# cure-lab/MotionCraft

Measured on AMD Instinct MI355X. Metric: sampled SMPL-X frames/sec (196-frame seq, 1000-step DDPM), higher is better.
Workload: dtype f32

## Files before the change

include/motioncraft_amd.h:

```cpp
#ifndef MOTIONCRAFT_AMD_H
#define MOTIONCRAFT_AMD_H
#include <stdint.h>

#ifdef __cplusplus
extern "C" {
#endif

#define MC_OK 0
#define MC_ERR_ARG 1
#define MC_ERR_HIP 2
#define MC_ERR_STATE 3
#define MC_ERR_NOCONV 4

typedef struct mc_model mc_model;
typedef struct mc_ctx mc_ctx;

typedef struct mc_model_config {
    int32_t input_feats;
    int32_t max_seq_len;
    int32_t latent_dim;
    int32_t num_parts;
    int32_t num_layers;
    int32_t ffn_dim;
    int32_t time_embed_dim;
// ... 116 lines not shown
int mc_op_temporal_attention(const float* mf_dev, const float* tf_dev, const float* mask_dev, float* yt_dev, int32_t b0, int32_t nb,
                             int32_t B, int32_t T, int32_t Nt, int32_t H, int32_t L, int32_t form, int32_t skip_text,
                             const int32_t* twin_flag_dev, void* stream);
enum { MC_ENC_ATTN_LAYER = 0,
       MC_ENC_ATTN_SMALL = 1,
       MC_ENC_ATTN_STREAM = 2 };
int mc_op_enc_ln(const float* x_dev, const float* gamma_dev, const float* beta_dev, float* y_dev, int64_t rows, int32_t L, float eps,
                 int32_t relu, void* stream);
int mc_op_enc_embed_tokens(const int32_t* ids_dev, const float* emb_dev, const float* pos_dev, float* x_dev, int64_t rows, int32_t S,
                           int32_t d, int32_t vocab, void* stream);
int mc_op_enc_attention(const float* qkv_dev, const uint8_t* valid_dev, float* out_dev, int32_t B, int32_t S, int32_t d, int32_t heads,
                        int32_t causal, int32_t form, void* stream);
enum { MC_GM_PLAIN = 0, MC_GM_ENC = 4 };
typedef struct mc_gemm_strided {
    const float* a_dev; int64_t lda, a_gstride;
    const float* w_dev; int64_t ldw, w_gstride;
    const float* bias_dev; int64_t b_gstride;
    float* c_dev; int64_t ldc, c_gstride;
    const float* res_dev; int64_t ldr, r_gstride;
    const float* add_dev; int64_t ld_add, dup_rows;
    int32_t add_mod, act, act_after_res, M, N, K;
} mc_gemm_strided;
int mc_op_gemm_strided(int32_t mode, int32_t groups, const mc_gemm_strided* args, void* stream);
int mc_op_bigru_steps(const float* gi_dev, const float* whh_dev, const float* bhh_dev, float* h_dev, const int32_t* lens_dev,
                      int32_t len_div, int32_t B, int32_t S, int32_t H, int32_t s0, int32_t steps, void* stream);
int mc_op_conv1d_k4s2(const float* x_dev, int64_t ldx, const float* w_tapmajor_dev, const float* bias_dev, float* y_padded_dev, int32_t B,
                      int32_t T, int32_t C, int32_t Cp, int32_t O, float slope, void* stream);
int mc_op_sampler_update(const float* x_t_dev, const float* out_text_dev, const float* out_none_dev,
                         const float* noise_dev, float* x_prev_dev, float* x0_dev, int64_t n,
                         const mc_step_coefs* coefs, void* stream);

#define MC_POST_MAXTAP 129
int mc_postprocess_smplx(const float* pred_dev, const int32_t* lengths_dev, const double* mean_dev,
                         const double* std_dev, const double* taps_dev, const int32_t radius[4], int32_t stats_f32,
                         int32_t B, int32_t T, int32_t C, double* poses_dev, double* expr_dev, double* trans_dev,
                         void* stream);
int mc_postprocess_smplx_stitched(const float* pred_dev, const int32_t* rows_dev, int32_t n_frames,
                                  const double* mean_dev, const double* std_dev, const double* taps_dev,
                                  const int32_t radius[4], int32_t stats_f32, int32_t C, double* poses_dev,
                                  double* expr_dev, double* trans_dev, void* stream);

int mc_postprocess_t2m_joints(const float* pred_dev, const int32_t* lengths_dev, const double* mean_dev,
                              const double* std_dev, const double* taps_dev, int32_t radius, int32_t stats_f32,
                              int32_t B, int32_t T, int32_t C, int32_t joints_num, float* joints_out_dev, void* stream);
int mc_postprocess_t2m_joints_stitched(const float* pred_dev, const int32_t* rows_dev, int32_t n_frames,
                                       const double* mean_dev, const double* std_dev, const double* taps_dev,
// ... 204 lines not shown
```

motioncraft_amd/csrc/mc_ctx.h:

```cpp
#pragma once
#include <map>
#include <mutex>
#include <string>
#include <vector>

#include "../../include/motioncraft_amd.h"
#include "mc_common.h"
#include "mc_gemm.h"
#include "mc_kernels.h"
#include "mc_chain.h"
#include "mc_half.h"
#include "mc_options.h"
#include "mc_params.h"

struct mc_model {
    mc_model_config cfg;
    ParamStore params{""};
    std::map<std::string, HalfW> half;
    std::mutex half_mu;
    size_t half_bytes = 0;
    bool finalized = false;
    int Cp = 0;
};

struct MoeW {
    const float *emb, *gate_w, *gate_b, *sim_n, *sim_nT, *scale, *fc1_w, *fc1_b, *fc2_wt, *fc2_b, *proj_w, *proj_b;
    int din, dout;
};

struct LayerW {
    const float *norm_g, *norm_b, *tnorm_g, *tnorm_b, *wsm;
    MoeW mm, tm;
    const float *dyn_g, *dyn_b, *qkv_w, *qkv_b;
    const float *ca_film_w, *ca_film_b, *ca_ln_g, *ca_ln_b, *ca_out_w, *ca_out_b;
    const float *ffn_w1, *ffn_b1, *ffn_w2, *ffn_b2;
    const float *ffn_film_w, *ffn_film_b, *ffn_ln_g, *ffn_ln_b, *ffn_out_w, *ffn_out_b;
    const float *before_w = nullptr, *before_b = nullptr, *after_w = nullptr, *after_b = nullptr;
    HalfW h_ca_out, h_ffn_out, h_fc1, h_fc2, h_w1, h_w2, h_after, h_proj, h_qkv;
};

struct ProfRec { hipEvent_t e0 = nullptr, e1 = nullptr; long rows = 0; };

struct mc_ctx {
    mc_model* m = nullptr;
    McOptions opt{};
// ... 80 lines not shown
```

motioncraft_amd/csrc/mc_gemm.h:

```cpp
#pragma once
#include <hip/hip_runtime.h>
#include "mc_options.h"
#include "../../include/motioncraft_amd.h"

enum { GM_PLAIN = MC_GM_PLAIN, GM_EXP1 = 1, GM_EXP2 = 2, GM_COMB = 3, GM_ENC = MC_GM_ENC };

enum : int {
    kTuneStaging = 1 << 0,
    kTuneDma = 1 << 4,
    kTuneWp = 1 << 5,
    kTuneNoXcd = 1 << 6,
    kTuneSmallXcd = 1 << 8,
    kTuneEncWp = 1 << 9,
    kTuneTail2 = 1 << 10,
    kTuneBits = kTuneStaging | kTuneDma | kTuneWp | kTuneNoXcd | kTuneSmallXcd | kTuneEncWp | kTuneTail2,
    kTuneDefault = kTuneBits & ~kTuneNoXcd,
};
static_assert(kTuneDefault == 1841, "the default tune bits are public ABI");

struct GemmArgs {
    const float* A = nullptr;
    long lda = 0;
    int a_col = 0;
    long a_gstride = 0;
    const float* W = nullptr;
    long ldw = 0;
    long w_gstride = 0;
    const float* bias = nullptr;
    long b_gstride = 0;
    float* C = nullptr;
    long ldc = 0;
    int c_col = 0;
    long c_gstride = 0;
    const float* R = nullptr;
    long ldr = 0;
    long r_gstride = -1;
    int act = 0;
    int act_after_res = 0;
    const float* add = nullptr;
    int add_mod = 1;
    long ld_add = 0;
    long dup_rows = 0;
    int M = 0, N = 0, K = 0;
    const int* tile_group = nullptr;
    const int* tile_row0 = nullptr;
    const int* tile_nrows = nullptr;
    const int* num_tiles = nullptr;
    const int* src_row = nullptr;
    const int* dst_row = nullptr;
    const float* comb_w = nullptr;
    int small_tile_n = 0;
    int wp_grid = 0;
    int tune = -1;
};

inline void mc_gemm_opts(const McOptions& o, GemmArgs& g) {
    g.tune = (int)o.gemm_tune;
    g.small_tile_n = o.small_tile_n ? (int)o.small_tile_n : -1;
    g.wp_grid = o.gemm_wp_grid > 0 ? (int)o.gemm_wp_grid : -1;
}

inline double mc_cu_load(long workgroups) {
    const long n = (workgroups + 255) / 256;
    return (1.45 * (double)(n / 2) + (double)(n % 2));
}

int mc_device_cus();
int mc_launch_gemm(int mode, const GemmArgs& g, int groups, int max_tiles, hipStream_t stream);
int mc_launch_gemm_small(const GemmArgs& g, hipStream_t stream, int groups = 1);

struct TailArgs {
    const float* H = nullptr;
    const float* Af = nullptr;
    long half = 0, lda = 0;
    const float* W = nullptr;
    long ldw = 0, w_gstride = 0;
    const float* bias = nullptr;
    long b_gstride = 0;
    float* C = nullptr;
    float* C2 = nullptr;
    long ldc = 0;
    int M = 0, N = 0, K = 0;
    float wc = 1.f, wu = 0.f;
    const float* coef_table = nullptr;
    const int* step_ptr = nullptr;
    long coef_stride = 0;
    int tune = -1;
};
int mc_launch_gemm_tail(const TailArgs& g, hipStream_t stream);
bool mc_gemm_tail_two_outputs(const TailArgs& g);
// ... 1 lines not shown
```

motioncraft_amd/csrc/mc_gemm.hip:

```cpp
#include "mc_common.h"
#include "mc_gemm.h"

namespace {

constexpr int BM = 128, BN = 128, BK = 32, LD = BK + 4;

struct Stage {
    long aoff[4], woff[4];
    bool aok[4], wok[4];
    float cw0[4], cw1[4];
};

template <int MODE, bool GUARD>
__device__ __forceinline__ void load_tile(const GemmArgs& g, const float* __restrict__ Ab, const float* __restrict__ Wb,
                                          const Stage& st, int k, f32x4 (&ra)[4], f32x4 (&rb)[4]) {
    const bool kin = !GUARD || k < g.K;
#pragma unroll
    for (int i = 0; i < 4; ++i) {
        f32x4 v = {0.f, 0.f, 0.f, 0.f};
        if ((!GUARD || st.aok[i]) && kin) {
            if constexpr (MODE == GM_COMB) {
                f32x4 y0 = {0.f, 0.f, 0.f, 0.f}, y1 = {0.f, 0.f, 0.f, 0.f};
                if (st.cw0[i] != 0.f) y0 = *reinterpret_cast<const f32x4*>(Ab + st.aoff[i] + k);
                if (st.cw1[i] != 0.f) y1 = *reinterpret_cast<const f32x4*>(Ab + st.aoff[i] + g.lda + k);
// ... 312 lines not shown
        const float* At = As + buf * BM * BK + (wm * 64 + frow) * BK;
        const float* Bt = Bs + buf * BN * BK + (wn * 64 + frow) * BK;
        Frag f0 = ld_frag(At, Bt, 0);
        Frag f1 = ld_frag(At, Bt, 1);
        __builtin_amdgcn_sched_barrier(0);
        mma(f0);
        f0 = ld_frag(At, Bt, 2);
        __builtin_amdgcn_sched_barrier(0);
        mma(f1);
        f1 = ld_frag(At, Bt, 3);
        __builtin_amdgcn_sched_barrier(0);
        mma(f0);
        mma(f1);
        __syncthreads();
    }
    if (g.act == ACT_GELU) epilogue_vec<GM_PLAIN, false, ACT_GELU>(g, 0, row0, BM, tn, wm, wn, lane, acc);
    else if (g.act == ACT_SILU) epilogue_vec<GM_PLAIN, false, ACT_SILU>(g, 0, row0, BM, tn, wm, wn, lane, acc);
    else if (g.act == ACT_NONE) epilogue_vec<GM_PLAIN, false, ACT_NONE>(g, 0, row0, BM, tn, wm, wn, lane, acc);
    else epilogue_vec<GM_PLAIN, false, ACT_LRELU>(g, 0, row0, BM, tn, wm, wn, lane, acc);
}

constexpr int WBK = 16, WSTAGE = 128 * WBK;

__global__ __launch_bounds__(256, 2) void gemm_wp_k(GemmArgs g) {
    __shared__ __attribute__((aligned(16))) float smem[4 * 2 * WSTAGE];
    const int tid = threadIdx.x, lane = tid & 63, wave = tid >> 6;
    const int wm = wave >> 1, wn = wave & 1;
    const int ntn = g.N / BN, ntiles = (g.M / BM) * ntn;
    const int wave_u = __builtin_amdgcn_readfirstlane(wave);
    float* wbase = smem + wave_u * 2 * WSTAGE;
    const unsigned lds0 = (unsigned)(size_t)wbase;
    const int dr = lane >> 2, dc = ((lane & 3) ^ ((dr >> 2) & 3)) * 4;
    const int frow = lane & 31, hf = lane >> 5, sw = (frow >> 2) & 3;
    const float* Ab = g.A + g.a_col;
    const float* Wb = g.W;
    const float* __restrict__ Rb = g.R ? g.R + g.c_col : nullptr;
    float* __restrict__ Cb = g.C + g.c_col;
    const int nk = g.K / WBK;
    struct Frag { f32x4 a0, a1, b0, b1; };
    auto ld_frag = [&](int st, int j) {
        const float* S = wbase + st * WSTAGE + frow * WBK + ((2 * j + hf) ^ sw) * 4;
        Frag f;
        f.a0 = *reinterpret_cast<const f32x4*>(S);
        f.a1 = *reinterpret_cast<const f32x4*>(S + 32 * WBK);
        f.b0 = *reinterpret_cast<const f32x4*>(S + 64 * WBK);
        f.b1 = *reinterpret_cast<const f32x4*>(S + 96 * WBK);
        return f;
    };
    for (int t = blockIdx.x; t < ntiles; t += gridDim.x) {
        const int bid = (g.tune & kTuneNoXcd) ? t : xcd_remap(t, ntiles);
        const int tm = bid / ntn, tn = bid % ntn;
        const int row0 = tm * BM;
        unsigned voa[4], vow[4];
#pragma unroll
        for (int q = 0; q < 4; ++q) {
            voa[q] = (unsigned)(((long)(row0 + wm * 64 + 16 * q + dr) * g.lda + dc) * 4);
            vow[q] = (unsigned)(((long)(tn * BN + wn * 64 + 16 * q + dr) * g.ldw + dc) * 4);
        }
        auto issue_q = [&](int kt, int st, int q) {
            const unsigned l = lds0 + st * WSTAGE * 4;
            dma16(voa[q], Ab + kt * WBK, l + q * 1024);
            dma16(vow[q], Wb + kt * WBK, l + 4096 + q * 1024);
        };
        f32x16 acc[2][2];
#pragma unroll
        for (int mi = 0; mi < 2; ++mi)
#pragma unroll
            for (int ni = 0; ni < 2; ++ni)
#pragma unroll
                for (int r = 0; r < 16; ++r) acc[mi][ni][r] = 0.f;
        auto mma2 = [&](const Frag& f, int i0) {
#pragma unroll
            for (int i = i0; i < i0 + 2; ++i) {
                acc[0][0] = __builtin_amdgcn_mfma_f32_32x32x2f32(f.b0[i], f.a0[i], acc[0][0], 0, 0, 0);
                acc[0][1] = __builtin_amdgcn_mfma_f32_32x32x2f32(f.b1[i], f.a0[i], acc[0][1], 0, 0, 0);
                acc[1][0] = __builtin_amdgcn_mfma_f32_32x32x2f32(f.b0[i], f.a1[i], acc[1][0], 0, 0, 0);
                acc[1][1] = __builtin_amdgcn_mfma_f32_32x32x2f32(f.b1[i], f.a1[i], acc[1][1], 0, 0, 0);
            }
        };
#pragma unroll
        for (int q = 0; q < 4; ++q) issue_q(0, 0, q);
        asm volatile("s_waitcnt vmcnt(0)" ::: "memory");
        Frag f0 = ld_frag(0, 0);
        auto ktile = [&](int kt) {
            const int st = kt & 1;
            const bool more = kt + 1 < nk;
            Frag f1 = ld_frag(st, 1);
            __builtin_amdgcn_sched_barrier(0);
            mma2(f0, 0);
            if (more) { issue_q(kt + 1, st ^ 1, 0); issue_q(kt + 1, st ^ 1, 1); }
            __builtin_amdgcn_sched_barrier(0);
            mma2(f0, 2);
            if (more) { issue_q(kt + 1, st ^ 1, 2); issue_q(kt + 1, st ^ 1, 3); }
            __builtin_amdgcn_sched_barrier(0);
            mma2(f1, 0);
            if (more) {
                asm volatile("s_waitcnt vmcnt(0)" ::: "memory");
                f0 = ld_frag(st ^ 1, 0);
            }
            __builtin_amdgcn_sched_barrier(0);
            mma2(f1, 2);
        };
        const int npre = nk > 2 ? nk - 2 : 0;
        for (int kt = 0; kt < npre; ++kt) ktile(kt);
        f32x4 rv[2][2][4], bv[2][4];
#pragma unroll
        for (int ni = 0; ni < 2; ++ni)
#pragma unroll
            for (int q = 0; q < 4; ++q) {
                const int n = tn * BN + wn * 64 + ni * 32 + 8 * q + 4 * hf;
                bv[ni][q] = g.bias ? *reinterpret_cast<const f32x4*>(g.bias + n) : f32x4{0.f, 0.f, 0.f, 0.f};
#pragma unroll
                for (int mi = 0; mi < 2; ++mi) {
                    const long m = row0 + wm * 64 + mi * 32 + frow;
                    rv[mi][ni][q] = Rb ? *reinterpret_cast<const f32x4*>(Rb + m * g.ldr + n) : f32x4{0.f, 0.f, 0.f, 0.f};
                    if (g.add) rv[mi][ni][q] = *reinterpret_cast<const f32x4*>(g.add + (m % g.add_mod) * g.ld_add + n);
                }
            }
        for (int kt = npre; kt < nk; ++kt) ktile(kt);
#pragma unroll
        for (int mi = 0; mi < 2; ++mi) {
            float* crow = Cb + (long)(row0 + wm * 64 + mi * 32 + frow) * g.ldc;
#pragma unroll
            for (int ni = 0; ni < 2; ++ni)
#pragma unroll
                for (int q = 0; q < 4; ++q) {
                    const int n = tn * BN + wn * 64 + ni * 32 + 8 * q + 4 * hf;
                    f32x4 v = {acc[mi][ni][4 * q], acc[mi][ni][4 * q + 1], acc[mi][ni][4 * q + 2], acc[mi][ni][4 * q + 3]};
                    v += bv[ni][q];
                    if (g.act != ACT_NONE) {
#pragma unroll
                        for (int jj = 0; jj < 4; ++jj) v[jj] = apply_act(v[jj], g.act);
                    }
                    v += rv[mi][ni][q];
                    *reinterpret_cast<f32x4*>(crow + n) = v;
                    if (g.dup_rows) *reinterpret_cast<f32x4*>(crow + g.dup_rows * g.ldc + n) = v;
                }
        }
    }
}

constexpr int SM = 64, SN = 64, SRING = 4;
template <bool VEC>
__global__ __launch_bounds__(256) void gemm_small_k(GemmArgs g) {
    __shared__ __attribute__((aligned(16))) float smem[SRING * 2 * SM * BK];
    const int tid = threadIdx.x, lane = tid & 63, wave = tid >> 6;
    const int wm = wave >> 1, wn = wave & 1;
    const int ntn = (g.N + SN - 1) / SN;
    const int bid = (g.tune & kTuneSmallXcd) ? xcd_remap((int)blockIdx.x, (int)gridDim.x) : (int)blockIdx.x;
    const int tm = bid / ntn, tn = bid % ntn, grp = blockIdx.y;
    const int row0 = tm * SM;
    const int wave_u = __builtin_amdgcn_readfirstlane(wave);
    const int dr = lane >> 3, dc = ((lane & 7) ^ dr) * 4;
    const float* Ab = g.A + (long)grp * g.a_gstride + g.a_col;
    const float* Wb = g.W + (long)grp * g.w_gstride;
    unsigned voa[2], vow[2];
#pragma unroll
    for (int q = 0; q < 2; ++q) {
        const int ar = min(row0 + 16 * wave + 8 * q + dr, g.M - 1), wr = min(tn * SN + 16 * wave + 8 * q + dr, g.N - 1);
        voa[q] = (unsigned)(((long)ar * g.lda + dc) * 4);
        vow[q] = (unsigned)(((long)wr * g.ldw + dc) * 4);
    }
// ... 510 lines not shown
    int nb = SN;
    double best = cost(SN, 30.0);
    const bool any_width = g.M > 6400;
    if ((g.N % 48 == 0 || any_width) && cost(48, 23.0) < 0.97 * best) { nb = 48; best = cost(48, 23.0); }
    if ((g.N % 96 == 0 || any_width) && cost(96, 41.0) < 0.97 * best) { nb = 96; best = cost(96, 41.0); }
    if (gg.small_tile_n == 64 || gg.small_tile_n == 48 || gg.small_tile_n == 96) nb = gg.small_tile_n;
    dim3 grid(cdiv(g.M, SM) * cdiv(g.N, nb), ng);
    const bool vec16 = vec && g.N % nb == 0;
    MC_LEDGER(nb == 48 ? "gemm_small16_k<3" : nb == 96 ? "gemm_small16_k<6" : "gemm_small_k", grid, 2.0 * g.M * g.N * g.K * ng);
    if (nb == 48) {
        if (vec16) hipLaunchKernelGGL((gemm_small16_k<3, true>), grid, dim3(256), 0, stream, gg);
        else hipLaunchKernelGGL((gemm_small16_k<3, false>), grid, dim3(256), 0, stream, gg);
    } else if (nb == 96) {
        if (vec16) hipLaunchKernelGGL((gemm_small16_k<6, true>), grid, dim3(256), 0, stream, gg);
        else hipLaunchKernelGGL((gemm_small16_k<6, false>), grid, dim3(256), 0, stream, gg);
    } else {
        if (vec) hipLaunchKernelGGL(gemm_small_k<true>, grid, dim3(256), 0, stream, gg);
        else hipLaunchKernelGGL(gemm_small_k<false>, grid, dim3(256), 0, stream, gg);
    }
    MC_LAUNCH_CHECK();
    return MC_OK;
}

int mc_launch_gemm(int mode, const GemmArgs& g0, int groups, int max_tiles, hipStream_t stream) {
    GemmArgs g = g0;
    if (int r = resolve_opts(g)) return r;
    const int ntn = cdiv(g.N, BN);
    int ntm = (mode == GM_EXP1 || mode == GM_EXP2) ? max_tiles : cdiv(g.M, BM);
    if (ntm <= 0 || ntn <= 0) return MC_OK;
    if (mode != GM_ENC) MC_REQUIRE(g.K % 4 == 0 && g.lda % 4 == 0 && g.ldw % 4 == 0, "gemm: K/lda/ldw must be multiples of 4");
    if (mode == GM_ENC && (g.add || g.dup_rows))
        MC_REQUIRE(g.N % 4 == 0 && g.ldc % 4 == 0 && g.c_col % 4 == 0 && g.c_gstride % 4 == 0 && (!g.add || g.ld_add % 4 == 0) &&
                       (!g.R || (g.ldr % 4 == 0 && (g.r_gstride < 0 || g.r_gstride % 4 == 0))),
                   "gemm: an add table or duplicate rows need 16-byte aligned output rows (N=%d ldc=%ld)", g.N, g.ldc);
    dim3 grid(ntm * ntn, groups > 0 ? groups : 1, 1);
    const bool vec_out = (g.ldc % 4 == 0) && (g.c_col % 4 == 0) && (!g.R || g.ldr % 4 == 0);
    const bool wp_ok = (g.tune & kTuneWp) && g.K % WBK == 0 && (long)g.M * g.lda * 4 < (1L << 32) && (long)g.N * g.ldw * 4 < (1L << 32);
    const bool enc_fast = mode == GM_ENC && (g.tune & kTuneEncWp) && wp_ok && !g.R && g.add && g.ld_add % 4 == 0 && g.act == ACT_NONE;
    if ((g.tune & kTuneDma) && (mode == GM_PLAIN || enc_fast) && groups <= 1 && g.M % BM == 0 && g.N % BN == 0 && (g.K % BK == 0 || enc_fast) &&
        g.lda % 4 == 0 && g.ldw % 4 == 0 && g.a_col % 4 == 0 && vec_out && g.act != ACT_QUICKGELU && !g.act_after_res &&
        (enc_fast || (!g.add && !g.dup_rows))) {
        if (wp_ok) {
            const int persistent = g.wp_grid > 0 ? g.wp_grid : (int)grid.x;
            MC_LEDGER("gemm_wp_k", dim3(grid.x < persistent ? grid.x : persistent), 2.0 * g.M * g.N * g.K);
            hipLaunchKernelGGL(gemm_wp_k, dim3(grid.x < persistent ? grid.x : persistent), dim3(256), 0, stream, g);
        } else {
            MC_LEDGER("gemm_dma_k", grid, 2.0 * g.M * g.N * g.K);
            hipLaunchKernelGGL(gemm_dma_k, grid, dim3(256), 0, stream, g);
        }
        MC_LAUNCH_CHECK();
        return MC_OK;
    }
    if (mc_ledger_on) {
        char name[24];
        snprintf(name, sizeof(name), "gemm_k<%d>", mode);
        const double rows = (mode == GM_EXP1 || mode == GM_EXP2) ? (double)ntm * BM : (double)g.M;
        MC_LEDGER(name, grid, 2.0 * rows * g.N * g.K * (groups > 0 ? groups : 1));
    }
    switch (mode) {
        case GM_PLAIN: hipLaunchKernelGGL(gemm_k<GM_PLAIN>, grid, dim3(256), 0, stream, g); break;
        case GM_EXP1: hipLaunchKernelGGL(gemm_k<GM_EXP1>, grid, dim3(256), 0, stream, g); break;
        case GM_EXP2: hipLaunchKernelGGL(gemm_k<GM_EXP2>, grid, dim3(256), 0, stream, g); break;
        case GM_COMB: hipLaunchKernelGGL(gemm_k<GM_COMB>, grid, dim3(256), 0, stream, g); break;
        case GM_ENC: hipLaunchKernelGGL(gemm_k<GM_ENC>, grid, dim3(256), 0, stream, g); break;
        default: mc_set_error("bad gemm mode %d", mode); return MC_ERR_ARG;
    }
    MC_LAUNCH_CHECK();
// ... 75 lines not shown
```

motioncraft_amd/csrc/mc_model.hip:

```cpp
#include "mc_ctx.h"

namespace {

template <class T>
int ws_alloc(mc_ctx* c, T** p, size_t n) {
    void* d = nullptr;
    size_t bytes = (n * sizeof(T) + 255) & ~(size_t)255;
    if (bytes == 0) bytes = 256;
    MC_HIP(hipMalloc(&d, bytes));
    c->allocs.push_back(d);
    c->bytes += (int64_t)bytes;
    *p = (T*)d;
    return MC_OK;
}

int bind_moe(const mc_model* m, const std::string& pre, int din, int dout, int seq_rows, MoeW* w) {
    const int64_t E = m->cfg.num_experts;
    w->din = din;
    w->dout = dout;
    return m->params.bind({{&w->emb, pre + "emb", (int64_t)seq_rows * din},       {&w->gate_w, pre + "gate_w", 256 * din},
                           {&w->gate_b, pre + "gate_b", 256},                      {&w->sim_n, pre + "sim_n", 256 * E},
                           {&w->sim_nT, pre + "sim_nT", 32 * 256},                 {&w->scale, pre + "scale", 1},
                           {&w->fc1_w, pre + "fc1_w", E * 4 * din * din},          {&w->fc1_b, pre + "fc1_b", E * 4 * din},
                           {&w->fc2_wt, pre + "fc2_wt", E * din * 4 * din},        {&w->fc2_b, pre + "fc2_b", E * din},
// ... 216 lines not shown
    MC_REQUIRE(cfg && out, "null argument");
    MC_REQUIRE(cfg->latent_dim == 32 || cfg->latent_dim == 64 || cfg->latent_dim == 128,
               "latent_dim=%d unsupported (32, 64, 128)", cfg->latent_dim);
    MC_REQUIRE(cfg->topk == 2, "topk=%d unsupported (reference configs use 2)", cfg->topk);
    MC_REQUIRE(cfg->num_experts >= 2 && cfg->num_experts <= 16, "num_experts=%d unsupported", cfg->num_experts);
    MC_REQUIRE(cfg->latent_dim % cfg->dyn_heads == 0, "latent_dim %% dyn_heads != 0");
    MC_REQUIRE(cfg->num_ctrl_layers >= 0 && cfg->num_ctrl_layers < cfg->num_layers, "copy_blocks_num=%d must be in [0, num_layers)", cfg->num_ctrl_layers);
    MC_REQUIRE(cfg->num_ctrl_layers == 0 || cfg->ctrl_cond_feats >= 1, "ctrl_cond_feats must be >= 1");
    MC_REQUIRE(cfg->ffn_dim % 4 == 0 && cfg->time_embed_dim % 4 == 0 && cfg->text_latent_dim % 4 == 0, "dims must be multiples of 4");
    {
        const int q = cfg->text_latent_dim / 4;
        MC_REQUIRE(q >= 1 && q <= 64 && (q & (q - 1)) == 0, "text_latent_dim=%d unsupported", cfg->text_latent_dim);
    }
    mc_model* m = new mc_model();
    m->cfg = *cfg;
    m->Cp = (cfg->input_feats + 31) / 32 * 32;
    *out = m;
    return MC_OK;
}

void mc_model_destroy(mc_model* m) {
    if (!m) return;
    for (auto& kv : m->half) (void)hipFree(const_cast<mc_half*>(kv.second.hi));
    delete m;
}

int mc_model_set_param(mc_model* m, const char* name, const float* host, int64_t numel) {
    MC_REQUIRE(m && name && host && numel > 0, "bad argument");
    MC_REQUIRE(!m->finalized || !m->params.has(name), "mc_model_set_param(%s): the model is finalized; weights are immutable from then on", name);
    return m->params.set(name, host, numel);
}

int mc_model_finalize(mc_model* m) {
    MC_REQUIRE(m, "null model");
    mc_ctx probe;
    probe.m = m;
    int r = bind_weights(&probe);
    if (r != MC_OK) return r;
    m->finalized = true;
    return MC_OK;
}

int mc_ctx_create(mc_model* m, int32_t batch, int32_t frames, int32_t max_steps, mc_ctx** out) {
    MC_REQUIRE(m && out, "null argument");
    MC_REQUIRE(m->finalized, "model not finalized");
    MC_REQUIRE(batch >= 1 && frames >= 1 && frames <= m->cfg.max_seq_len, "bad batch/frames (%d, %d)", batch, frames);
    MC_REQUIRE(max_steps >= 1, "max_steps < 1");
    const mc_model_config& g = m->cfg;
    mc_ctx* c = new mc_ctx();
    if (int r = seed_options(c->opt)) { mc_ctx_destroy(c); return r; }
    c->m = m;
    c->B = batch;
    c->T = frames;
// ... 484 lines not shown
int mc_op_gemm(const float* a, const float* w, const float* bias, const float* res, float* cdev, int32_t M, int32_t N,
               int32_t K, int32_t ldw, int32_t act, void* stream) {
    MC_REQUIRE(a && w && cdev && M > 0 && N > 0 && K > 0 && K % 4 == 0 && ldw % 4 == 0 && ldw >= K, "bad gemm args");
    return dense(nullptr, a, K, w, ldw, bias, res, N, cdev, N, M, N, K, act, (hipStream_t)stream);
}

int mc_op_gemm_strided(int32_t mode, int32_t groups, const mc_gemm_strided* a, void* stream) {
    MC_REQUIRE(a && (mode == GM_PLAIN || mode == GM_ENC) && groups >= 1, "gemm_strided: mode %d (0 plain, 4 encoder), groups %d", mode, groups);
    MC_REQUIRE(a->a_dev && a->w_dev && a->c_dev && a->M > 0 && a->N > 0 && a->K > 0 && a->lda > 0 && a->ldc >= a->N && a->ldw >= a->K &&
                   a->ldw % 4 == 0 && a->add_mod >= 1 && a->dup_rows >= 0 && (!a->res_dev || a->ldr >= a->N) && (!a->add_dev || a->ld_add >= a->N),
               "bad gemm_strided args");
    GemmArgs g;
    g.A = a->a_dev; g.lda = a->lda; g.a_gstride = a->a_gstride;
    g.W = a->w_dev; g.ldw = a->ldw; g.w_gstride = a->w_gstride;
    g.bias = a->bias_dev; g.b_gstride = a->b_gstride;
    g.C = a->c_dev; g.ldc = a->ldc; g.c_gstride = a->c_gstride;
    g.R = a->res_dev; g.ldr = a->ldr; g.r_gstride = a->r_gstride;
    g.act = a->act; g.act_after_res = a->act_after_res;
    g.add = a->add_dev; g.add_mod = a->add_mod; g.ld_add = a->ld_add; g.dup_rows = a->dup_rows;
    g.M = a->M; g.N = a->N; g.K = a->K;
    return mc_launch_gemm(mode, g, groups, 0, (hipStream_t)stream);
}

static int gemm_f16_op(GemmHArgs g, const float* w, const float* bias, const float* res, float* cdev, int M, int N, int K, bool split, hipStream_t s) {
    mc_half* planes = nullptr;
    MC_HIP(hipMalloc((void**)&planes, sizeof(mc_half) * 2 * (size_t)N * K));
    int r = mc_launch_split_f16(w, planes, planes + (size_t)N * K, (long)N * K, s);
    if (r == MC_OK) {
        g.Wh = planes; g.Wl = planes + (size_t)N * K; g.bias = bias; g.R = res; g.ldr = N; g.C = cdev; g.ldc = N;
        g.M = M; g.N = N; g.K = K;
        r = mc_launch_gemm_h(g, split, s);
    }
    (void)hipStreamSynchronize(s);
    (void)hipFree(planes);
    return r;
}

int mc_op_gemm_f16(const float* a, const float* w, const float* bias, const float* res, float* cdev, int32_t M, int32_t N,
                   int32_t K, int32_t split, void* stream) {
    MC_REQUIRE(a && w && cdev && M > 0 && N > 0 && K > 0, "bad gemm args");
    GemmHArgs g;
    g.A = a; g.lda = K;
    return gemm_f16_op(g, w, bias, res, cdev, M, N, K, split != 0, (hipStream_t)stream);
}

int mc_op_gemm_f16_planes(const void* a_hi, const void* a_lo, const float* w, const float* bias, const float* res, float* cdev, int32_t M,
// ... 80 lines not shown
```

motioncraft_amd/csrc/mc_step.hip:

```cpp
#include "mc_ctx.h"

bool use_half(const mc_ctx* c) { return c->prec != MC_PREC_F32 && c->rows > c->opt.half_min_rows; }
static const HalfW* half_planes(const mc_ctx* c, const HalfW* hw) { return hw && hw->hi && use_half(c) ? hw : nullptr; }
static bool split3(const mc_ctx* c) { return c->prec == MC_PREC_F16X3; }

static bool twin_aliased(const mc_ctx* c, bool twin) { return twin && chain_on(c, kChainTwinAlias) && !c->no_alias; }
static TwinAlias twin_alias(const mc_ctx* c, bool twin, bool tokens) {
    return twin_aliased(c, twin) ? TwinAlias{mc_route_split_flag_ptr(c->rb), (tokens ? c->N : c->rows) / 2} : TwinAlias();
}

template <class Args>
static void set_tile_map(const mc_ctx* c, int group, Args& a) {
    const long to = (long)group * c->rb.max_tiles;
    a.tile_group = c->rb.tile_group + to; a.tile_row0 = c->rb.tile_row0 + to; a.tile_nrows = c->rb.tile_nrows + to;
    a.num_tiles = mc_route_num_tiles_ptr(c->rb, group);
}

static int dbg_hold(const mc_ctx* c, hipStream_t pos, hipStream_t neg) {
    const long us = c->opt.dbg_delay_us;
    return us == 0 ? MC_OK : mc_launch_spin((us > 0 ? us : -us) * 100, us > 0 ? pos : neg);
}

int dense(const mc_ctx* c, const float* A, long lda, const float* W, long ldw, const float* bias, const float* R, long ldr,
          float* C, long ldc, long M, int N, int K, int act, hipStream_t s) {
// ... 474 lines not shown
int denoise_impl(mc_ctx* c, const float* x_t, int32_t step, float* out2_dev, int32_t stop_after, void* stream, const SeedArgs* seed) {
    MC_REQUIRE(c && x_t, "null argument");
    MC_REQUIRE(c->have_cond, "mc_ctx_set_condition not called");
    MC_REQUIRE(step >= 0 && step < c->S, "step_index %d outside the %d-step schedule", step, c->S);
    if (c->graph_mode) step = 0;
    hipStream_t s = (hipStream_t)stream;
    const mc_model_config& g = c->m->cfg;
    const int L = g.latent_dim, H = g.num_parts, D = L * H, C = g.input_feats;
    const long BT = (long)c->B * c->T;
    int r;
    if ((r = pick_side_stream(c, s))) return r;
    {
        const bool padded = c->xpad_ready && !seed;
        c->xpad_ready = false;
        if (seed) { if ((r = mc_launch_pad_rows_seeded(const_cast<float*>(x_t), c->xpad, BT, C, c->m->Cp, *seed, s))) return r; }
        else if (!padded && (r = mc_launch_pad_rows(x_t, c->xpad, BT, C, c->m->Cp, s))) return r;
        GemmArgs e;
        mc_gemm_opts(c->opt, e);
        e.A = c->xpad; e.lda = c->m->Cp;
        e.W = c->enc_w; e.ldw = c->m->Cp; e.bias = c->enc_b;
        e.add = c->seq_emb; e.add_mod = c->T; e.ld_add = D;
        e.C = c->h; e.ldc = D; e.dup_rows = BT;
        e.M = (int)BT; e.N = D; e.K = c->m->Cp;
        if (BT <= c->opt.small_gemm_rows && D % 64 == 0 && c->m->Cp % 32 == 0) { if ((r = mc_launch_gemm_small(e, s))) return r; }
        else if ((r = mc_launch_gemm(GM_ENC, e, 1, 0, s))) return r;
    }
    const int nl = stop_after >= 0 ? (stop_after < g.num_layers ? stop_after : g.num_layers) : g.num_layers;
    c->no_alias = stop_after >= 0 && stop_after < g.num_layers;
    const int NC = c->have_ctrl ? g.num_ctrl_layers : 0;
    const bool fused = chain_on(c, kChainGate) && chain_on(c, kChainRowchain) && mc_mlp_supported(L, 32);
    const int split = (c->side && chain_on(c, kChainTwoStreams) && c->N > c->opt.big_tokens && fused) ? ((NC > 0 && !chain_on(c, kChainCtrlGroups)) ? 1 : 2) : 0;
    auto by_group = [&](auto&& fn) -> int {
        if (split != 2) return fn(0L, c->rows, s);
        if (int e = fn(0L, BT, s)) return e;
        return fn(BT, BT, c->side);
    };
    for (int i = 0; i < nl; ++i) {
        if (i >= 1 && i <= NC) {
            const int j = i - 1, slot = g.num_layers + j;
            if (j == 0) {
                if ((r = by_group([&](long r0, long n, hipStream_t sk) {
                         return mc_launch_add_rows(c->hc + r0 * D, c->h + r0 * D, c->cb + r0 * D, nullptr, n, D, sk); })))
                    return r;
            }
            if ((r = run_layer(c, slot, c->hc, step, false, split, s))) return r;
            const LayerW& cw = c->lw[slot];
            if ((r = by_group([&](long r0, long n, hipStream_t sk) {
// ... 80 lines not shown
```

Before: 661.1.

## Skip all-zero weight K-tiles in encoder GEMM and split remainder tiles in half

```diff
diff --git a/include/motioncraft_amd.h b/include/motioncraft_amd.h
--- a/include/motioncraft_amd.h
+++ b/include/motioncraft_amd.h
@@ -162,6 +162,7 @@
     int32_t add_mod, act, act_after_res, M, N, K;
 } mc_gemm_strided;
 int mc_op_gemm_strided(int32_t mode, int32_t groups, const mc_gemm_strided* args, void* stream);
+int mc_op_gemm_wp(int32_t mode, const mc_gemm_strided* args, int32_t wp_grid, int64_t tune, int32_t klist, void* stream);
 int mc_op_bigru_steps(const float* gi_dev, const float* whh_dev, const float* bhh_dev, float* h_dev, const int32_t* lens_dev,
                       int32_t len_div, int32_t B, int32_t S, int32_t H, int32_t s0, int32_t steps, void* stream);
 int mc_op_conv1d_k4s2(const float* x_dev, int64_t ldx, const float* w_tapmajor_dev, const float* bias_dev, float* y_padded_dev, int32_t B,
diff --git a/motioncraft_amd/csrc/mc_ctx.h b/motioncraft_amd/csrc/mc_ctx.h
--- a/motioncraft_amd/csrc/mc_ctx.h
+++ b/motioncraft_amd/csrc/mc_ctx.h
@@ -21,6 +21,7 @@
     size_t half_bytes = 0;
     bool finalized = false;
     int Cp = 0;
+    int* enc_klist = nullptr;
 };
 
 struct MoeW {
diff --git a/motioncraft_amd/csrc/mc_gemm.h b/motioncraft_amd/csrc/mc_gemm.h
--- a/motioncraft_amd/csrc/mc_gemm.h
+++ b/motioncraft_amd/csrc/mc_gemm.h
@@ -1,5 +1,6 @@
 #pragma once
 #include <hip/hip_runtime.h>
+#include <vector>
 #include "mc_options.h"
 #include "../../include/motioncraft_amd.h"
 
@@ -13,10 +14,12 @@
     kTuneSmallXcd = 1 << 8,
     kTuneEncWp = 1 << 9,
     kTuneTail2 = 1 << 10,
-    kTuneBits = kTuneStaging | kTuneDma | kTuneWp | kTuneNoXcd | kTuneSmallXcd | kTuneEncWp | kTuneTail2,
+    kTuneEncSkip = 1 << 11,
+    kTuneHalfTiles = 1 << 12,
+    kTuneBits = kTuneStaging | kTuneDma | kTuneWp | kTuneNoXcd | kTuneSmallXcd | kTuneEncWp | kTuneTail2 | kTuneEncSkip | kTuneHalfTiles,
     kTuneDefault = kTuneBits & ~kTuneNoXcd,
 };
-static_assert(kTuneDefault == 1841, "the default tune bits are public ABI");
+static_assert(kTuneDefault == 7985, "the default tune bits are public ABI");
 
 struct GemmArgs {
     const float* A = nullptr;
@@ -49,6 +52,7 @@
     const int* src_row = nullptr;
     const int* dst_row = nullptr;
     const float* comb_w = nullptr;
+    const int* klist = nullptr;
     int small_tile_n = 0;
     int wp_grid = 0;
     int tune = -1;
@@ -66,6 +70,8 @@
 }
 
 int mc_device_cus();
+std::vector<int> mc_gemm_klist(const float* w_host, int N, int K, long ldw);
+bool mc_gemm_takes_wp(int mode, const GemmArgs& g, int groups);
 int mc_launch_gemm(int mode, const GemmArgs& g, int groups, int max_tiles, hipStream_t stream);
 int mc_launch_gemm_small(const GemmArgs& g, hipStream_t stream, int groups = 1);
 
diff --git a/motioncraft_amd/csrc/mc_gemm.hip b/motioncraft_amd/csrc/mc_gemm.hip
--- a/motioncraft_amd/csrc/mc_gemm.hip
+++ b/motioncraft_amd/csrc/mc_gemm.hip
@@ -358,6 +358,124 @@
 
 constexpr int WBK = 16, WSTAGE = 128 * WBK;
 
+template <int MI, bool LIST>
+__device__ __forceinline__ void wp_tile(const GemmArgs& g, float* wbase, int row0, int tn, const int* __restrict__ kl, int lane, int wm, int wn) {
+    const unsigned lds0 = (unsigned)(size_t)wbase;
+    const int dr = lane >> 2, dc = ((lane & 3) ^ ((dr >> 2) & 3)) * 4;
+    const int frow = lane & 31, hf = lane >> 5, sw = (frow >> 2) & 3;
+    const float* Ab = g.A + g.a_col;
+    const float* Wb = g.W;
+    const float* __restrict__ Rb = !LIST && g.R ? g.R + g.c_col : nullptr;
+    float* __restrict__ Cb = g.C + g.c_col;
+    const int nk = LIST ? kl[0] : g.K / WBK;
+    auto kcol = [&](int i) { return (LIST ? kl[1 + i] : i) * WBK; };
+    const int wrow = row0 + wm * 32 * MI;
+    struct Frag { f32x4 a[MI], b[2]; };
+    auto ld_frag = [&](int st, int j) {
+        const float* S = wbase + st * WSTAGE + frow * WBK + ((2 * j + hf) ^ sw) * 4;
+        Frag f;
+#pragma unroll
+        for (int mi = 0; mi < MI; ++mi) f.a[mi] = *reinterpret_cast<const f32x4*>(S + 32 * mi * WBK);
+#pragma unroll
+        for (int ni = 0; ni < 2; ++ni) f.b[ni] = *reinterpret_cast<const f32x4*>(S + (64 + 32 * ni) * WBK);
+        return f;
+    };
+    unsigned voa[2 * MI], vow[4];
+#pragma unroll
+    for (int q = 0; q < 4; ++q) {
+        if (q < 2 * MI) voa[q] = (unsigned)(((long)(wrow + 16 * q + dr) * g.lda + dc) * 4);
+        vow[q] = (unsigned)(((long)(tn * BN + wn * 64 + 16 * q + dr) * g.ldw + dc) * 4);
+    }
+    auto issue_q = [&](int kc, int st, int q) {
+        const unsigned l = lds0 + st * WSTAGE * 4;
+        if (q < 2 * MI) dma16(voa[q], Ab + kc, l + q * 1024);
+        dma16(vow[q], Wb + kc, l + 4096 + q * 1024);
+    };
+    f32x16 acc[MI][2];
+#pragma unroll
+    for (int mi = 0; mi < MI; ++mi)
+#pragma unroll
+        for (int ni = 0; ni < 2; ++ni)
+#pragma unroll
+            for (int r = 0; r < 16; ++r) acc[mi][ni][r] = 0.f;
+    auto mma2 = [&](const Frag& f, int i0) {
+#pragma unroll
+        for (int i = i0; i < i0 + 2; ++i)
+#pragma unroll
+            for (int mi = 0; mi < MI; ++mi)
+#pragma unroll
+                for (int ni = 0; ni < 2; ++ni)
+                    acc[mi][ni] = __builtin_amdgcn_mfma_f32_32x32x2f32(f.b[ni][i], f.a[mi][i], acc[mi][ni], 0, 0, 0);
+    };
+    if (!LIST || nk > 0) {
+        const int kc = kcol(0);
+#pragma unroll
+        for (int q = 0; q < 4; ++q) issue_q(kc, 0, q);
+    }
+    asm volatile("s_waitcnt vmcnt(0)" ::: "memory");
+    Frag f0;
+    if (!LIST || nk > 0) f0 = ld_frag(0, 0);
+    auto ktile = [&](int kt) {
+        const int st = kt & 1;
+        const bool more = kt + 1 < nk;
+        const int kc = more ? kcol(kt + 1) : 0;
+        Frag f1 = ld_frag(st, 1);
+        __builtin_amdgcn_sched_barrier(0);
+        mma2(f0, 0);
+        if (more) {
+            issue_q(kc, st ^ 1, 0); issue_q(kc, st ^ 1, 1);
+            if (MI == 1) { issue_q(kc, st ^ 1, 2); issue_q(kc, st ^ 1, 3); }
+        }
+        __builtin_amdgcn_sched_barrier(0);
+        mma2(f0, 2);
+        if (more && MI == 2) { issue_q(kc, st ^ 1, 2); issue_q(kc, st ^ 1, 3); }
+        __builtin_amdgcn_sched_barrier(0);
+        mma2(f1, 0);
+        if (more) {
+            asm volatile("s_waitcnt vmcnt(0)" ::: "memory");
+            f0 = ld_frag(st ^ 1, 0);
+        }
+        __builtin_amdgcn_sched_barrier(0);
+        mma2(f1, 2);
+    };
+    const int npre = nk > 2 ? nk - 2 : 0;
+    for (int kt = 0; kt < npre; ++kt) ktile(kt);
+    f32x4 rv[MI][2][4], bv[2][4];
+#pragma unroll
+    for (int ni = 0; ni < 2; ++ni)
+#pragma unroll
+        for (int q = 0; q < 4; ++q) {
+            const int n = tn * BN + wn * 64 + ni * 32 + 8 * q + 4 * hf;
+            bv[ni][q] = g.bias ? *reinterpret_cast<const f32x4*>(g.bias + n) : f32x4{0.f, 0.f, 0.f, 0.f};
+#pragma unroll
+            for (int mi = 0; mi < MI; ++mi) {
+                const long m = wrow + mi * 32 + frow;
+                rv[mi][ni][q] = Rb ? *reinterpret_cast<const f32x4*>(Rb + m * g.ldr + n) : f32x4{0.f, 0.f, 0.f, 0.f};
+                if (g.add) rv[mi][ni][q] = *reinterpret_cast<const f32x4*>(g.add + (m % g.add_mod) * g.ld_add + n);
+            }
+        }
+    for (int kt = npre; kt < nk; ++kt) ktile(kt);
+#pragma unroll
+    for (int mi = 0; mi < MI; ++mi) {
+        float* crow = Cb + (long)(wrow + mi * 32 + frow) * g.ldc;
+#pragma unroll
+        for (int ni = 0; ni < 2; ++ni)
+#pragma unroll
+            for (int q = 0; q < 4; ++q) {
+                const int n = tn * BN + wn * 64 + ni * 32 + 8 * q + 4 * hf;
+                f32x4 v = {acc[mi][ni][4 * q], acc[mi][ni][4 * q + 1], acc[mi][ni][4 * q + 2], acc[mi][ni][4 * q + 3]};
+                v += bv[ni][q];
+                if (!LIST && g.act != ACT_NONE) {
+#pragma unroll
+                    for (int jj = 0; jj < 4; ++jj) v[jj] = apply_act(v[jj], g.act);
+                }
+                v += rv[mi][ni][q];
+                *reinterpret_cast<f32x4*>(crow + n) = v;
+                if (g.dup_rows) *reinterpret_cast<f32x4*>(crow + g.dup_rows * g.ldc + n) = v;
+            }
+    }
+}
+
 __global__ __launch_bounds__(256, 2) void gemm_wp_k(GemmArgs g) {
     __shared__ __attribute__((aligned(16))) float smem[4 * 2 * WSTAGE];
     const int tid = threadIdx.x, lane = tid & 63, wave = tid >> 6;
@@ -365,115 +483,25 @@
     const int ntn = g.N / BN, ntiles = (g.M / BM) * ntn;
     const int wave_u = __builtin_amdgcn_readfirstlane(wave);
     float* wbase = smem + wave_u * 2 * WSTAGE;
-    const unsigned lds0 = (unsigned)(size_t)wbase;
-    const int dr = lane >> 2, dc = ((lane & 3) ^ ((dr >> 2) & 3)) * 4;
-    const int frow = lane & 31, hf = lane >> 5, sw = (frow >> 2) & 3;
-    const float* Ab = g.A + g.a_col;
-    const float* Wb = g.W;
-    const float* __restrict__ Rb = g.R ? g.R + g.c_col : nullptr;
-    float* __restrict__ Cb = g.C + g.c_col;
-    const int nk = g.K / WBK;
-    struct Frag { f32x4 a0, a1, b0, b1; };
-    auto ld_frag = [&](int st, int j) {
-        const float* S = wbase + st * WSTAGE + frow * WBK + ((2 * j + hf) ^ sw) * 4;
-        Frag f;
-        f.a0 = *reinterpret_cast<const f32x4*>(S);
-        f.a1 = *reinterpret_cast<const f32x4*>(S + 32 * WBK);
-        f.b0 = *reinterpret_cast<const f32x4*>(S + 64 * WBK);
-        f.b1 = *reinterpret_cast<const f32x4*>(S + 96 * WBK);
-        return f;
-    };
-    for (int t = blockIdx.x; t < ntiles; t += gridDim.x) {
+    const int nkl = g.K / WBK + 1;
+    const int G = gridDim.x, b = blockIdx.x;
+    const int rem = ntiles % G;
+    const bool halves = (g.tune & kTuneHalfTiles) && rem > 0 && 2 * rem <= G && !g.klist;
+    const int whole = halves ? ntiles - rem : ntiles;
+    for (int t = b; t < whole; t += G) {
         const int bid = (g.tune & kTuneNoXcd) ? t : xcd_remap(t, ntiles);
         const int tm = bid / ntn, tn = bid % ntn;
-        const int row0 = tm * BM;
-        unsigned voa[4], vow[4];
-#pragma unroll
-        for (int q = 0; q < 4; ++q) {
-            voa[q] = (unsigned)(((long)(row0 + wm * 64 + 16 * q + dr) * g.lda + dc) * 4);
-            vow[q] = (unsigned)(((long)(tn * BN + wn * 64 + 16 * q + dr) * g.ldw + dc) * 4);
-        }
-        auto issue_q = [&](int kt, int st, int q) {
-            const unsigned l = lds0 + st * WSTAGE * 4;
-            dma16(voa[q], Ab + kt * WBK, l + q * 1024);
-            dma16(vow[q], Wb + kt * WBK, l + 4096 + q * 1024);
-        };
-        f32x16 acc[2][2];
-#pragma unroll
-        for (int mi = 0; mi < 2; ++mi)
-#pragma unroll
-            for (int ni = 0; ni < 2; ++ni)
-#pragma unroll
-                for (int r = 0; r < 16; ++r) acc[mi][ni][r] = 0.f;
-        auto mma2 = [&](const Frag& f, int i0) {
-#pragma unroll
-            for (int i = i0; i < i0 + 2; ++i) {
-                acc[0][0] = __builtin_amdgcn_mfma_f32_32x32x2f32(f.b0[i], f.a0[i], acc[0][0], 0, 0, 0);
-                acc[0][1] = __builtin_amdgcn_mfma_f32_32x32x2f32(f.b1[i], f.a0[i], acc[0][1], 0, 0, 0);
-                acc[1][0] = __builtin_amdgcn_mfma_f32_32x32x2f32(f.b0[i], f.a1[i], acc[1][0], 0, 0, 0);
-                acc[1][1] = __builtin_amdgcn_mfma_f32_32x32x2f32(f.b1[i], f.a1[i], acc[1][1], 0, 0, 0);
-            }
-        };
-#pragma unroll
-        for (int q = 0; q < 4; ++q) issue_q(0, 0, q);
-        asm volatile("s_waitcnt vmcnt(0)" ::: "memory");
-        Frag f0 = ld_frag(0, 0);
-        auto ktile = [&](int kt) {
-            const int st = kt & 1;
-            const bool more = kt + 1 < nk;
-            Frag f1 = ld_frag(st, 1);
-            __builtin_amdgcn_sched_barrier(0);
-            mma2(f0, 0);
-            if (more) { issue_q(kt + 1, st ^ 1, 0); issue_q(kt + 1, st ^ 1, 1); }
-            __builtin_amdgcn_sched_barrier(0);
-            mma2(f0, 2);
-            if (more) { issue_q(kt + 1, st ^ 1, 2); issue_q(kt + 1, st ^ 1, 3); }
-            __builtin_amdgcn_sched_barrier(0);
-            mma2(f1, 0);
-            if (more) {
-                asm volatile("s_waitcnt vmcnt(0)" ::: "memory");
-                f0 = ld_frag(st ^ 1, 0);
-            }
-            __builtin_amdgcn_sched_barrier(0);
-            mma2(f1, 2);
-        };
-        const int npre = nk > 2 ? nk - 2 : 0;
-        for (int kt = 0; kt < npre; ++kt) ktile(kt);
-        f32x4 rv[2][2][4], bv[2][4];
-#pragma unroll
-        for (int ni = 0; ni < 2; ++ni)
-#pragma unroll
-            for (int q = 0; q < 4; ++q) {
-                const int n = tn * BN + wn * 64 + ni * 32 + 8 * q + 4 * hf;
-                bv[ni][q] = g.bias ? *reinterpret_cast<const f32x4*>(g.bias + n) : f32x4{0.f, 0.f, 0.f, 0.f};
-#pragma unroll
-                for (int mi = 0; mi < 2; ++mi) {
-                    const long m = row0 + wm * 64 + mi * 32 + frow;
-                    rv[mi][ni][q] = Rb ? *reinterpret_cast<const f32x4*>(Rb + m * g.ldr + n) : f32x4{0.f, 0.f, 0.f, 0.f};
-                    if (g.add) rv[mi][ni][q] = *reinterpret_cast<const f32x4*>(g.add + (m % g.add_mod) * g.ld_add + n);
-                }
-            }
-        for (int kt = npre; kt < nk; ++kt) ktile(kt);
-#pragma unroll
-        for (int mi = 0; mi < 2; ++mi) {
-            float* crow = Cb + (long)(row0 + wm * 64 + mi * 32 + frow) * g.ldc;
-#pragma unroll
-            for (int ni = 0; ni < 2; ++ni)
-#pragma unroll
-                for (int q = 0; q < 4; ++q) {
-                    const int n = tn * BN + wn * 64 + ni * 32 + 8 * q + 4 * hf;
-                    f32x4 v = {acc[mi][ni][4 * q], acc[mi][ni][4 * q + 1], acc[mi][ni][4 * q + 2], acc[mi][ni][4 * q + 3]};
-                    v += bv[ni][q];
-                    if (g.act != ACT_NONE) {
-#pragma unroll
-                        for (int jj = 0; jj < 4; ++jj) v[jj] = apply_act(v[jj], g.act);
-                    }
-                    v += rv[mi][ni][q];
-                    *reinterpret_cast<f32x4*>(crow + n) = v;
-                    if (g.dup_rows) *reinterpret_cast<f32x4*>(crow + g.dup_rows * g.ldc + n) = v;
-                }
-        }
-    }
+        if (g.klist) wp_tile<2, true>(g, wbase, tm * BM, tn, g.klist + tn * nkl, lane, wm, wn);
+        else wp_tile<2, false>(g, wbase, tm * BM, tn, nullptr, lane, wm, wn);
+    }
+    if (!halves) return;
+    const bool by_xcd = G % 16 == 0;
+    const int j = by_xcd ? (b >> 4) * 8 + (b & 7) : b >> 1, hi = by_xcd ? (b >> 3) & 1 : b & 1;
+    if (j >= rem) return;
+    const int t = whole + j;
+    const int bid = (g.tune & kTuneNoXcd) ? t : xcd_remap(t, ntiles);
+    const int tm = bid / ntn, tn = bid % ntn;
+    wp_tile<1, false>(g, wbase, tm * BM + 64 * hi, tn, nullptr, lane, wm, wn);
 }
 
 constexpr int SM = 64, SN = 64, SRING = 4;
@@ -1030,6 +1058,33 @@
     return MC_OK;
 }
 
+struct DmaForm { bool dma, wp, enc_fast; };
+static DmaForm dma_form(int mode, const GemmArgs& g, int groups) {
+    const bool vec_out = (g.ldc % 4 == 0) && (g.c_col % 4 == 0) && (!g.R || g.ldr % 4 == 0);
+    const bool wp_ok = (g.tune & kTuneWp) && g.K % WBK == 0 && (long)g.M * g.lda * 4 < (1L << 32) && (long)g.N * g.ldw * 4 < (1L << 32);
+    const bool enc_fast = mode == GM_ENC && (g.tune & kTuneEncWp) && wp_ok && !g.R && g.add && g.ld_add % 4 == 0 && g.act == ACT_NONE;
+    const bool dma = (g.tune & kTuneDma) && (mode == GM_PLAIN || enc_fast) && groups <= 1 && g.M % BM == 0 && g.N % BN == 0 &&
+                     (g.K % BK == 0 || enc_fast) && g.lda % 4 == 0 && g.ldw % 4 == 0 && g.a_col % 4 == 0 && vec_out && g.act != ACT_QUICKGELU &&
+                     !g.act_after_res && (enc_fast || (!g.add && !g.dup_rows));
+    return {dma, dma && wp_ok, enc_fast};
+}
+bool mc_gemm_takes_wp(int mode, const GemmArgs& g, int groups) { return g.M > 0 && g.N > 0 && dma_form(mode, g, groups).wp; }
+
+std::vector<int> mc_gemm_klist(const float* w, int N, int K, long ldw) {
+    const int ntn = N / BN, nk = K / WBK;
+    std::vector<int> kl((size_t)ntn * (nk + 1), 0);
+    for (int tn = 0; tn < ntn; ++tn) {
+        int* row = kl.data() + (size_t)tn * (nk + 1);
+        for (int kt = 0; kt < nk; ++kt) {
+            bool any = false;
+            for (int n = tn * BN; n < (tn + 1) * BN && !any; ++n)
+                for (int k = kt * WBK; k < (kt + 1) * WBK && !any; ++k) any = !(w[(long)n * ldw + k] == 0.0f);
+            if (any) row[1 + row[0]++] = kt;
+        }
+    }
+    return kl;
+}
+
 int mc_launch_gemm(int mode, const GemmArgs& g0, int groups, int max_tiles, hipStream_t stream) {
     GemmArgs g = g0;
     if (int r = resolve_opts(g)) return r;
@@ -1042,15 +1097,11 @@
                        (!g.R || (g.ldr % 4 == 0 && (g.r_gstride < 0 || g.r_gstride % 4 == 0))),
                    "gemm: an add table or duplicate rows need 16-byte aligned output rows (N=%d ldc=%ld)", g.N, g.ldc);
     dim3 grid(ntm * ntn, groups > 0 ? groups : 1, 1);
-    const bool vec_out = (g.ldc % 4 == 0) && (g.c_col % 4 == 0) && (!g.R || g.ldr % 4 == 0);
-    const bool wp_ok = (g.tune & kTuneWp) && g.K % WBK == 0 && (long)g.M * g.lda * 4 < (1L << 32) && (long)g.N * g.ldw * 4 < (1L << 32);
-    const bool enc_fast = mode == GM_ENC && (g.tune & kTuneEncWp) && wp_ok && !g.R && g.add && g.ld_add % 4 == 0 && g.act == ACT_NONE;
-    if ((g.tune & kTuneDma) && (mode == GM_PLAIN || enc_fast) && groups <= 1 && g.M % BM == 0 && g.N % BN == 0 && (g.K % BK == 0 || enc_fast) &&
-        g.lda % 4 == 0 && g.ldw % 4 == 0 && g.a_col % 4 == 0 && vec_out && g.act != ACT_QUICKGELU && !g.act_after_res &&
-        (enc_fast || (!g.add && !g.dup_rows))) {
-        if (wp_ok) {
+    const DmaForm form = dma_form(mode, g, groups);
+    if (form.dma) {
+        if (form.wp) {
             const int persistent = g.wp_grid > 0 ? g.wp_grid : (int)grid.x;
-            MC_LEDGER("gemm_wp_k", dim3(grid.x < persistent ? grid.x : persistent), 2.0 * g.M * g.N * g.K);
+            if (!(form.enc_fast && (g.tune & kTuneEncSkip))) g.klist = nullptr;            MC_LEDGER("gemm_wp_k", dim3(grid.x < persistent ? grid.x : persistent), 2.0 * g.M * g.N * g.K);
             hipLaunchKernelGGL(gemm_wp_k, dim3(grid.x < persistent ? grid.x : persistent), dim3(256), 0, stream, g);
         } else {
             MC_LEDGER("gemm_dma_k", grid, 2.0 * g.M * g.N * g.K);
diff --git a/motioncraft_amd/csrc/mc_model.hip b/motioncraft_amd/csrc/mc_model.hip
--- a/motioncraft_amd/csrc/mc_model.hip
+++ b/motioncraft_amd/csrc/mc_model.hip
@@ -262,13 +262,25 @@
 void mc_model_destroy(mc_model* m) {
     if (!m) return;
     for (auto& kv : m->half) (void)hipFree(const_cast<mc_half*>(kv.second.hi));
+    if (m->enc_klist) (void)hipFree(m->enc_klist);
     delete m;
+}
+
+static int rebuild_enc_klist(mc_model* m, const float* host, int64_t numel) {
+    if (m->enc_klist) { (void)hipFree(m->enc_klist); m->enc_klist = nullptr; }
+    const int D = m->cfg.latent_dim * m->cfg.num_parts;
+    if (D % 128 != 0 || numel != (int64_t)D * m->Cp) return MC_OK;
+    const std::vector<int> kl = mc_gemm_klist(host, D, m->Cp, m->Cp);
+    MC_HIP(hipMalloc((void**)&m->enc_klist, kl.size() * sizeof(int)));
+    MC_HIP(hipMemcpy(m->enc_klist, kl.data(), kl.size() * sizeof(int), hipMemcpyHostToDevice));
+    return MC_OK;
 }
 
 int mc_model_set_param(mc_model* m, const char* name, const float* host, int64_t numel) {
     MC_REQUIRE(m && name && host && numel > 0, "bad argument");
     MC_REQUIRE(!m->finalized || !m->params.has(name), "mc_model_set_param(%s): the model is finalized; weights are immutable from then on", name);
-    return m->params.set(name, host, numel);
+    if (int r = m->params.set(name, host, numel)) return r;
+    return std::string(name) == "enc.w" ? rebuild_enc_klist(m, host, numel) : MC_OK;
 }
 
 int mc_model_finalize(mc_model* m) {
@@ -799,6 +811,45 @@
     return mc_launch_gemm(mode, g, groups, 0, (hipStream_t)stream);
 }
 
+int mc_op_gemm_wp(int32_t mode, const mc_gemm_strided* a, int32_t wp_grid, int64_t tune, int32_t klist, void* stream) {
+    MC_REQUIRE(a && (mode == GM_PLAIN || mode == GM_ENC), "gemm_wp: mode %d (0 plain, 4 encoder)", mode);
+    MC_REQUIRE(a->a_dev && a->w_dev && a->c_dev && a->M > 0 && a->N > 0 && a->K > 0 && a->lda >= a->K && a->ldc >= a->N && a->ldw >= a->K &&
+                   a->ldw % 4 == 0 && a->add_mod >= 1 && a->dup_rows >= 0 && (!a->res_dev || a->ldr >= a->N) && (!a->add_dev || a->ld_add >= a->N) &&
+                   wp_grid >= 1, "bad gemm_wp args");
+    const std::string why = check_tune((long)tune);
+    MC_REQUIRE(why.empty(), "%s", why.c_str());
+    const McOptions* o = mc_process_options();
+    if (!o) return MC_ERR_ARG;
+    GemmArgs g;
+    mc_gemm_opts(*o, g);
+    g.tune = (int)tune; g.wp_grid = wp_grid;
+    g.A = a->a_dev; g.lda = a->lda; g.W = a->w_dev; g.ldw = a->ldw; g.bias = a->bias_dev;
+    g.C = a->c_dev; g.ldc = a->ldc; g.R = a->res_dev; g.ldr = a->ldr;
+    g.act = a->act; g.act_after_res = a->act_after_res;
+    g.add = a->add_dev; g.add_mod = a->add_mod; g.ld_add = a->ld_add; g.dup_rows = a->dup_rows;
+    g.M = a->M; g.N = a->N; g.K = a->K;
+    MC_REQUIRE(mc_gemm_takes_wp(mode, g, 1), "gemm_wp: this launch does not run on gemm_wp_k (M, N %% 128, K %% 16 (plain: 32), tune bits 4 and 5, "
+               "encoder mode: tune bit 9 and an add table; M=%d N=%d K=%d tune=%ld)", a->M, a->N, a->K, (long)tune);
+    hipStream_t s = (hipStream_t)stream;
+    int* kl_dev = nullptr;
+    if (klist) {
+        std::vector<float> w((size_t)(a->N - 1) * a->ldw + a->K);
+        MC_HIP(hipStreamSynchronize(s));
+        MC_HIP(hipMemcpy(w.data(), a->w_dev, w.size() * sizeof(float), hipMemcpyDeviceToHost));
+        const std::vector<int> kl = mc_gemm_klist(w.data(), a->N, a->K, a->ldw);
+        MC_HIP(hipMalloc((void**)&kl_dev, kl.size() * sizeof(int)));
+        const hipError_t e = hipMemcpy(kl_dev, kl.data(), kl.size() * sizeof(int), hipMemcpyHostToDevice);
+        if (e != hipSuccess) { (void)hipFree(kl_dev); MC_HIP(e); }
+        g.klist = kl_dev;
+    }
+    const int r = mc_launch_gemm(mode, g, 1, 0, s);
+    if (kl_dev) {
+        (void)hipStreamSynchronize(s);
+        (void)hipFree(kl_dev);
+    }
+    return r;
+}
+
 static int gemm_f16_op(GemmHArgs g, const float* w, const float* bias, const float* res, float* cdev, int M, int N, int K, bool split, hipStream_t s) {
     mc_half* planes = nullptr;
     MC_HIP(hipMalloc((void**)&planes, sizeof(mc_half) * 2 * (size_t)N * K));
diff --git a/motioncraft_amd/csrc/mc_step.hip b/motioncraft_amd/csrc/mc_step.hip
--- a/motioncraft_amd/csrc/mc_step.hip
+++ b/motioncraft_amd/csrc/mc_step.hip
@@ -520,7 +520,8 @@
         e.add = c->seq_emb; e.add_mod = c->T; e.ld_add = D;
         e.C = c->h; e.ldc = D; e.dup_rows = BT;
         e.M = (int)BT; e.N = D; e.K = c->m->Cp;
-        if (BT <= c->opt.small_gemm_rows && D % 64 == 0 && c->m->Cp % 32 == 0) { if ((r = mc_launch_gemm_small(e, s))) return r; }
+        if (!use_half(c)) e.klist = c->m->enc_klist;
+        if (BT <=c->opt.small_gemm_rows && D % 64 == 0 && c->m->Cp % 32 == 0) { if ((r = mc_launch_gemm_small(e, s))) return r; }
         else if ((r = mc_launch_gemm(GM_ENC, e, 1, 0, s))) return r;
     }
     const int nl = stop_after >= 0 ? (stop_after < g.num_layers ? stop_after : g.num_layers) : g.num_layers;
```

After: 660.9. About the same (-0.0%).
